# hank-kuo-cs/Volumetric-Primitives-Net

Measured on NVIDIA B200. Metric: primitive-loss fwd+bwd samples/sec, higher is better.
Workload: dtype f32

## Files before the change

### volumetric-primitives-net_b200/csrc/chamfer_tiled.cu

```cuda
#include <cstdlib>
#include <mutex>
#include <type_traits>
#include "common.cuh"

namespace vpn {

enum { MODE_EXACT = 0, MODE_DIFF = 1, MODE_EXPAND = 2, MODE_TC = 3 };

constexpr int kTThreads = 256;
constexpr int kTWarps = kTThreads / 32;
constexpr int kCW = 128;
constexpr int kMaxChunksPerSplit = 64;
constexpr float kBig = 1.0e30f;

__device__ __forceinline__ u64 pk(float a, float b) { u64 r; asm("mov.b64 %0, {%1,%2};" : "=l"(r) : "f"(a), "f"(b)); return r; }
__device__ __forceinline__ void upk(u64 v, float& a, float& b) { asm("mov.b64 {%0,%1}, %2;" : "=f"(a), "=f"(b) : "l"(v)); }
__device__ __forceinline__ u64 add2(u64 a, u64 b) { u64 r; asm("add.rn.f32x2 %0, %1, %2;" : "=l"(r) : "l"(a), "l"(b)); return r; }
__device__ __forceinline__ u64 sub2(u64 a, u64 b) { u64 r; asm("sub.rn.f32x2 %0, %1, %2;" : "=l"(r) : "l"(a), "l"(b)); return r; }
__device__ __forceinline__ u64 mul2(u64 a, u64 b) { u64 r; asm("mul.rn.f32x2 %0, %1, %2;" : "=l"(r) : "l"(a), "l"(b)); return r; }
__device__ __forceinline__ u64 fma2(u64 a, u64 b, u64 c) { u64 r; asm("fma.rn.f32x2 %0, %1, %2, %3;" : "=l"(r) : "l"(a), "l"(b), "l"(c)); return r; }
__device__ __forceinline__ float min3f(float a, float b, float c) { float r; asm("min.f32 %0, %1, %2, %3;" : "=f"(r) : "f"(a), "f"(b), "f"(c)); return r; }
__device__ __forceinline__ float warp_min_f32(float a) { float r; asm volatile("redux.sync.min.f32 %0, %1, 0xffffffff;" : "=f"(r) : "f"(a)); return r; }
__device__ __forceinline__ float inf_f() { return __int_as_float(0x7f800000); }

__device__ __forceinline__ float thr_of(float x, float rel, float abs_) {
  return __fadd_ru(__fmaf_ru(fabsf(x), rel, x), abs_);
}
__device__ __forceinline__ float mode_rel(int mode) {
  return mode == MODE_EXACT ? 9.5367431640625e-07f
       : mode == MODE_DIFF ? 3.814697265625e-06f
                           : 3.0517578125e-05f;
}

__device__ __forceinline__ float exact_d2s(float ax, float ay, float az, float bx, float by, float bz) {
  float dx = __fsub_rn(ax, bx), dy = __fsub_rn(ay, by), dz = __fsub_rn(az, bz);
  return __fadd_rn(__fadd_rn(__fmul_rn(dx, dx), __fmul_rn(dy, dy)), __fmul_rn(dz, dz));
}

template <int R>
struct TiledSmem {
  float4 tile[2][kCW];
  float colw[2][kTWarps][kCW];
  float rs_best[R][kTThreads];
  float rs_thr[R][kTThreads];
  u64 rs_mask[R][kTThreads];
  float red[kTWarps][4];
  float ctr[4];
};

template <int MODE>
__device__ __forceinline__ u64 pair_val(u64 c0, u64 c1, u64 c2, u64 c3, const float4& col, float one) {
  if (MODE == MODE_EXPAND) {
    u64 e = fma2(c0, pk(col.x, col.x), c3);
    e = fma2(c1, pk(col.y, col.y), e);
    e = fma2(c2, pk(col.z, col.z), e);
    return add2(e, pk(col.w, col.w));
  }
  u64 dx = sub2(c0, pk(col.x, col.x)), dy = sub2(c1, pk(col.y, col.y)), dz = sub2(c2, pk(col.z, col.z));
  if (MODE == MODE_EXACT) {
    u64 xx = mul2(dx, dx), yy = mul2(dy, dy), zz = mul2(dz, dz);
    u64 o2 = pk(one, one);
    return fma2(fma2(xx, o2, yy), o2, zz);
  }
  return fma2(dz, dz, fma2(dy, dy, mul2(dx, dx)));
}

template <int R, int MODE>
__global__ void __launch_bounds__(kTThreads, (R <= 8 ? 2 : 1))
chamfer_tiled_kernel(const float* __restrict__ p1, const float* __restrict__ p2,
                     float* __restrict__ rbest, u64* __restrict__ rmask,
                     float* __restrict__ cbest, unsigned* __restrict__ cmask,
                     float2* __restrict__ tslack, int* __restrict__ fallback,
                     int P, int M, int nchunks, int cps, float one, int only_flagged) {
  constexpr int TM = kTThreads * R;
  extern __shared__ __align__(16) unsigned char smem_raw[];
  TiledSmem<R>& sm = *reinterpret_cast<TiledSmem<R>*>(smem_raw);
  const int tid = threadIdx.x, lane = tid & 31, warp = tid >> 5;
  const int tile_i = blockIdx.x, split = blockIdx.y, b = blockIdx.z;
  const int ntiles = gridDim.x, nsplit = gridDim.y;
  if (only_flagged && fallback[b] == 0) return;
  const float* A = p1 + (size_t)b * P * 3;
  const float* T = p2 + (size_t)b * M * 3;

  u64 c0[R / 2], c1[R / 2], c2[R / 2], c3[R / 2];
  float rm[R];
  float cx = 0.f, cy = 0.f, cz = 0.f;
  float slack_rel = mode_rel(MODE), slack_abs = 1e-36f;
  {
    float x[R], y[R], z[R];
#pragma unroll
    for (int r = 0; r < R; ++r) {
      int i = min(tile_i * TM + r * kTThreads + tid, P - 1);
      x[r] = A[3 * (size_t)i]; y[r] = A[3 * (size_t)i + 1]; z[r] = A[3 * (size_t)i + 2];
    }
    if (MODE == MODE_EXPAND) {
      float sx = 0.f, sy = 0.f, sz = 0.f;
#pragma unroll
      for (int r = 0; r < R; ++r) { sx += x[r]; sy += y[r]; sz += z[r]; }
      sx = warp_sum(sx); sy = warp_sum(sy); sz = warp_sum(sz);
      if (lane == 0) { sm.red[warp][0] = sx; sm.red[warp][1] = sy; sm.red[warp][2] = sz; }
      __syncthreads();
      if (tid < 3) {
        float s = 0.f;
#pragma unroll
        for (int w = 0; w < kTWarps; ++w) s += sm.red[w][tid];
        sm.ctr[tid] = s / (float)TM;
      }
      __syncthreads();
      cx = sm.ctr[0]; cy = sm.ctr[1]; cz = sm.ctr[2];
      float rho2 = 0.f;
#pragma unroll
      for (int r = 0; r < R; ++r) {
        x[r] = __fsub_rn(x[r], cx); y[r] = __fsub_rn(y[r], cy); z[r] = __fsub_rn(z[r], cz);
        rho2 = fmaxf(rho2, fmaf(z[r], z[r], fmaf(y[r], y[r], x[r] * x[r])));
      }
#pragma unroll
      for (int o = 16; o > 0; o >>= 1) rho2 = fmaxf(rho2, __shfl_xor_sync(0xffffffffu, rho2, o));
      __syncthreads();
      if (lane == 0) sm.red[warp][3] = rho2;
      __syncthreads();
      rho2 = sm.red[0][3];
#pragma unroll
      for (int w = 1; w < kTWarps; ++w) rho2 = fmaxf(rho2, sm.red[w][3]);
      if (!(rho2 < kBig)) { if (tid == 0) atomicOr(&fallback[b], 1); rho2 = 0.f; }
      slack_abs = __fmaf_ru(8.0e-5f, rho2, 1e-36f);
    }
#pragma unroll
    for (int rp = 0; rp < R / 2; ++rp) {
      const int r0 = 2 * rp, r1 = 2 * rp + 1;
      if (MODE == MODE_EXPAND) {
        c0[rp] = pk(-2.f * x[r0], -2.f * x[r1]); c1[rp] = pk(-2.f * y[r0], -2.f * y[r1]); c2[rp] = pk(-2.f * z[r0], -2.f * z[r1]);
        c3[rp] = pk(fmaf(z[r0], z[r0], fmaf(y[r0], y[r0], x[r0] * x[r0])), fmaf(z[r1], z[r1], fmaf(y[r1], y[r1], x[r1] * x[r1])));
      } else {
        c0[rp] = pk(x[r0], x[r1]); c1[rp] = pk(y[r0], y[r1]); c2[rp] = pk(z[r0], z[r1]); c3[rp] = 0ull;
      }
    }
  }
  if (tid == 0 && split == 0) tslack[(size_t)b * ntiles + tile_i] = make_float2(slack_rel, slack_abs);
#pragma unroll
  for (int r = 0; r < R; ++r) {
    rm[r] = inf_f();
    sm.rs_best[r][tid] = inf_f(); sm.rs_thr[r][tid] = inf_f(); sm.rs_mask[r][tid] = 0ull;
  }
  const int c_first = split * cps;
  const int c_last = min(nchunks, c_first + cps);

  auto make_col = [&](float tx, float ty, float tz) -> float4 {
    if (MODE == MODE_EXPAND) {
      float x = __fsub_rn(tx, cx), y = __fsub_rn(ty, cy), z = __fsub_rn(tz, cz);
      float c = fmaf(z, z, fmaf(y, y, x * x));
      if (!(c < kBig)) atomicOr(&fallback[b], 1);
      return make_float4(x, y, z, c);
    }
    return make_float4(tx, ty, tz, 0.f);
  };

  if (tid < kCW) {
    int col = min(c_first * kCW + tid, M - 1);
    sm.tile[0][tid] = make_col(T[3 * (size_t)col], T[3 * (size_t)col + 1], T[3 * (size_t)col + 2]);
  }
  __syncthreads();

  for (int c = c_first; c < c_last; ++c) {
    const int buf = (c - c_first) & 1;
    float nx = 0.f, ny = 0.f, nz = 0.f;
    const bool has_next = (c + 1 < c_last) && (tid < kCW);
    if (has_next) {
      int col = min((c + 1) * kCW + tid, M - 1);
      nx = T[3 * (size_t)col]; ny = T[3 * (size_t)col + 1]; nz = T[3 * (size_t)col + 2];
    }
    const float4* tl = sm.tile[buf];
    float* cw = sm.colw[buf][warp];
#pragma unroll 2
    for (int k = 0; k < kCW; k += 2) {
      const float4 q0 = tl[k], q1 = tl[k + 1];
      float cm0 = inf_f(), cm1 = inf_f();
#pragma unroll
      for (int rp = 0; rp < R / 2; ++rp) {
        u64 d0 = pair_val<MODE>(c0[rp], c1[rp], c2[rp], c3[rp], q0, one);
        u64 d1 = pair_val<MODE>(c0[rp], c1[rp], c2[rp], c3[rp], q1, one);
        float a0, b0, a1, b1;
        upk(d0, a0, b0); upk(d1, a1, b1);
        rm[2 * rp] = min3f(rm[2 * rp], a0, a1);
        rm[2 * rp + 1] = min3f(rm[2 * rp + 1], b0, b1);
        cm0 = min3f(cm0, a0, b0);
        cm1 = min3f(cm1, a1, b1);
      }
      float w0 = warp_min_f32(cm0), w1 = warp_min_f32(cm1);
      if (lane == 0) *reinterpret_cast<float2*>(cw + k) = make_float2(w0, w1);
    }
    const u64 bit = 1ull << (c - c_first);
#pragma unroll
    for (int r = 0; r < R; ++r) {
      const float m = rm[r];
      rm[r] = inf_f();
      if (m <= sm.rs_thr[r][tid]) {
        const float best = sm.rs_best[r][tid];
        const float tm = thr_of(m, slack_rel, slack_abs);
        u64 mask = (tm < best) ? 0ull : sm.rs_mask[r][tid];
        sm.rs_mask[r][tid] = mask | bit;
        if (m < best) { sm.rs_best[r][tid] = m; sm.rs_thr[r][tid] = tm; }
      }
    }
    if (has_next) sm.tile[buf ^ 1][tid] = make_col(nx, ny, nz);
    __syncthreads();
    if (tid < kCW) {
      const int col = c * kCW + tid;
      if (col < M) {
        float w[kTWarps];
        float best = inf_f();
#pragma unroll
        for (int i = 0; i < kTWarps; ++i) { w[i] = sm.colw[buf][i][tid]; best = fminf(best, w[i]); }
        const float t = thr_of(best, slack_rel, slack_abs);
        unsigned mask = 0;
#pragma unroll
        for (int i = 0; i < kTWarps; ++i) mask |= (w[i] <= t) ? (1u << i) : 0u;
        size_t o = ((size_t)b * ntiles + tile_i) * M + col;
        cbest[o] = best; cmask[o] = mask;
      }
    }
  }
#pragma unroll
  for (int r = 0; r < R; ++r) {
    int row = tile_i * TM + r * kTThreads + tid;
    if (row < P) {
      size_t o = ((size_t)b * nsplit + split) * P + row;
      rbest[o] = sm.rs_best[r][tid]; rmask[o] = sm.rs_mask[r][tid];
    }
  }
}

constexpr int kRecThreads = 1024;
constexpr int kSegChunks = 64;
constexpr int kItemCap = 4096;

struct ExactBest {
  float d, hi, v; int i;
  __device__ __forceinline__ void init() { d = inf_f(); hi = inf_f(); v = inf_f(); i = 0x7fffffff; }
  __device__ __forceinline__ void offer(float dd, int idx) {
    if (dd <= hi) {
      float vv = sqrtf(dd);
      if (vv < v || (vv == v && idx < i)) { v = vv; i = idx; }
      if (dd < d) { d = dd; hi = thr_of(dd, 9.5367431640625e-07f, 1e-36f); }
    }
  }
  __device__ __forceinline__ u64 key() const { return ((u64)__float_as_uint(v) << 32) | (unsigned)i; }
};

__device__ __forceinline__ int unit_scan(const float (&d)[32], float dm, int rot, int* at) {
  if (!(dm < inf_f())) {
    bool any = false;
#pragma unroll
    for (int kk = 0; kk < 32; ++kk) any |= (d[kk] == inf_f());
    if (!any) return 0;
    return 2;
  }
  const float hi = thr_of(dm, 9.5367431640625e-07f, 1e-36f);
  int cnt = 0, pos = 0;
#pragma unroll
  for (int kk = 0; kk < 32; ++kk) {
    const bool in = d[kk] <= hi;
    cnt += in ? 1 : 0;
    pos += in ? kk : 0;
  }
  *at = (pos + rot) & 31;
  return cnt == 1 ? 1 : 2;
}

__device__ __noinline__ u64 unit_exact_walk(float ax, float ay, float az, const float4* __restrict__ pts, int idx0, int use_w) {
  ExactBest eb; eb.init();
  for (int k = 0; k < 32; ++k) {
    const float4 q = pts[k];
    eb.offer(exact_d2s(ax, ay, az, q.x, q.y, q.z), use_w ? __float_as_int(q.w) : idx0 + k);
  }
  return eb.i != 0x7fffffff ? eb.key() : ~0ull;
}

template <int NT>
__device__ __forceinline__ int block_exclusive_scan(int cnt, int* warp_sums, int* total) {
  const int lane = threadIdx.x & 31, warp = threadIdx.x >> 5;
  int inc = cnt;
#pragma unroll
  for (int o = 1; o < 32; o <<= 1) { int t = __shfl_up_sync(0xffffffffu, inc, o); if (lane >= o) inc += t; }
  if (lane == 31) warp_sums[warp] = inc;
  __syncthreads();
  if (warp == 0) {
    int w = lane < NT / 32 ? warp_sums[lane] : 0;
    int winc = w;
#pragma unroll
    for (int o = 1; o < 32; o <<= 1) { int t = __shfl_up_sync(0xffffffffu, winc, o); if (lane >= o) winc += t; }
    warp_sums[lane] = winc - w;
    if (lane == 31) warp_sums[32] = winc;
  }
  __syncthreads();
  int off = warp_sums[warp] + inc - cnt;
  *total = warp_sums[32];
  __syncthreads();
  return off;
}

__device__ __forceinline__ u64 expand_chunk_bits16(unsigned v) {
  u64 x = v & 0xffffu;
  x = (x | (x << 24)) & 0x000000ff000000ffull;
  x = (x | (x << 12)) & 0x000f000f000f000full;
  x = (x | (x << 6)) & 0x0303030303030303ull;
  x = (x | (x << 3)) & 0x1111111111111111ull;
  return x * 0xfull;
}
__device__ __forceinline__ void or_shifted256(u64 (&seg)[4], u64 w, int base) {
  if (w == 0ull || base >= 256 || base <= -64) return;
  const int k = base >> 6, sh = base & 63;
#pragma unroll
  for (int kk = 0; kk < 4; ++kk) {
    if (kk == k) seg[kk] |= w << sh;
    if (sh != 0 && kk == k + 1) seg[kk] |= w >> (64 - sh);
  }
}

constexpr int kRowGroup = kRecThreads / 2;
constexpr int kRowItemCap = kItemCap / 2;
constexpr size_t kRowsFixedSmem = (size_t)kRecThreads * (16 + 8 + 32 + 4 + 12 + 4) + (size_t)kItemCap * 4;
__device__ __forceinline__ void group_sync(int bar) { asm volatile("bar.sync %0, %1;" :: "r"(bar), "n"(kRowGroup) : "memory"); }
__device__ __forceinline__ int group_exclusive_scan(int cnt, int* warp_sums, int* total, int gt, int bar) {
  const int lane = gt & 31, warp = gt >> 5;
  int inc = cnt;
#pragma unroll
  for (int o = 1; o < 32; o <<= 1) { int t = __shfl_up_sync(0xffffffffu, inc, o); if (lane >= o) inc += t; }
  if (lane == 31) warp_sums[warp] = inc;
  group_sync(bar);
  if (warp == 0) {
    int w = lane < kRowGroup / 32 ? warp_sums[lane] : 0;
    int winc = w;
#pragma unroll
    for (int o = 1; o < 32; o <<= 1) { int t = __shfl_up_sync(0xffffffffu, winc, o); if (lane >= o) winc += t; }
    if (lane < kRowGroup / 32) warp_sums[lane] = winc - w;
    if (lane == 31) warp_sums[kRowGroup / 32] = winc;
  }
  group_sync(bar);
  int off = warp_sums[warp] + inc - cnt;
  *total = warp_sums[kRowGroup / 32];
  group_sync(bar);
  return off;
}

__global__ void __launch_bounds__(kRecThreads, 1)
chamfer_recover_rows_kernel(const float* __restrict__ p1, const float* __restrict__ p2, const float4* __restrict__ p2v, int mpad,
                            const float* __restrict__ rbest, const u64* __restrict__ rmask, int planes, size_t plane_stride,
                            const float2* __restrict__ tslack, float* __restrict__ min1, int* __restrict__ idx1,
                            int P, int M, int nchunks, int nsplit, int cps, int TM, int ntiles,
                            const int* __restrict__ skip, int nblk, int nitems, const int* __restrict__ rperm) {
  extern __shared__ __align__(16) unsigned char smem_raw[];
  float4* rowc_ = reinterpret_cast<float4*>(smem_raw);
  u64* key_ = reinterpret_cast<u64*>(rowc_ + kRecThreads);
  u64 (*pre_mask)[kRecThreads] = reinterpret_cast<u64 (*)[kRecThreads]>(key_ + kRecThreads);
  unsigned* items_ = reinterpret_cast<unsigned*>(pre_mask + 4);
  float* pre_rb = reinterpret_cast<float*>(items_ + kItemCap);
  float* pre_p1 = pre_rb + kRecThreads;
  int* pre_perm = reinterpret_cast<int*>(pre_p1 + 3 * kRecThreads);
  float4* cols = reinterpret_cast<float4*>(smem_raw + kRowsFixedSmem);
  __shared__ int warp_sums_[2][kRowGroup / 32 + 1];
  const int tid = threadIdx.x, lane = tid & 31, grp = tid / kRowGroup, gt = tid % kRowGroup, bar = 1 + grp;
  const bool use_pre = (nsplit == 1) && (planes == 4);
  auto prefetch = [&](int b_, int wi_) {
    const int row_ = (wi_ - b_ * nblk) * kRowGroup + gt;
    if (row_ < P) {
      const size_t o_ = (size_t)b_ * P + row_;
      cp_async4(&pre_rb[tid], rbest + o_);
#pragma unroll
      for (int w = 0; w < 4; ++w) cp_async8(&pre_mask[w][tid], rmask + o_ + w * plane_stride);
#pragma unroll
      for (int k = 0; k < 3; ++k) cp_async4(&pre_p1[tid * 3 + k], p1 + 3 * o_ + k);
      if (rperm) cp_async4(&pre_perm[tid], rperm + o_);
    }
    asm volatile("cp.async.commit_group;" ::: "memory");
  };
  float4* rowc = rowc_ + grp * kRowGroup; u64* key = key_ + grp * kRowGroup;
  unsigned* items = items_ + grp * kRowItemCap; int* warp_sums = warp_sums_[grp];
  const int per = (nitems + gridDim.x - 1) / gridDim.x;
  const int w0 = blockIdx.x * per, w1 = min(nitems, w0 + per);
  const int nseg = (nchunks + kSegChunks - 1) / kSegChunks;
  const float qnan = __int_as_float(0x7fc00000);
  for (int b = w0 / nblk; b * nblk < w1; ++b) {
    if (skip && skip[b]) continue;
    const int i0 = max(w0, b * nblk), i1 = min(w1, (b + 1) * nblk);
    for (int seg = 0; seg < nseg; ++seg) {
      const int seg_chunks = min(kSegChunks, nchunks - seg * kSegChunks);
      __syncthreads();
      if (p2v) {
        const float4* src = p2v + (size_t)b * mpad + (size_t)seg * kSegChunks * kCW;
        for (int i = tid; i < seg_chunks * kCW; i += kRecThreads) cols[i] = src[i];
      } else {
        const float* T = p2 + (size_t)b * M * 3;
        for (int i = tid; i < seg_chunks * kCW; i += kRecThreads) {
          const int col = seg * kSegChunks * kCW + i;
          cols[i] = col < M ? make_float4(T[3 * (size_t)col], T[3 * (size_t)col + 1], T[3 * (size_t)col + 2], __int_as_float(col))
                            : make_float4(qnan, qnan, qnan, __int_as_float(0x7fffffff));
        }
      }
      __syncthreads();
      if (use_pre && i0 + grp < i1) prefetch(b, i0 + grp);
      for (int wi = i0 + grp; wi < i1; wi += 2) {
        const int row = (wi - b * nblk) * kRowGroup + gt;
        const bool valid = row < P;
        auto orow_of = [&]() { return (size_t)b * P + (use_pre ? __float_as_int(rowc[gt].w) : (rperm ? rperm[(size_t)b * P + row] : row)); };
        float g = inf_f(), gthr = inf_f();
        u64 kinit = ~0ull;
        u64 sg[4] = {0ull, 0ull, 0ull, 0ull};
        if (use_pre) {
          asm volatile("cp.async.wait_all;" ::: "memory");
          if (valid) {
            rowc[gt] = make_float4(pre_p1[tid * 3], pre_p1[tid * 3 + 1], pre_p1[tid * 3 + 2], __int_as_float(rperm ? pre_perm[tid] : row));
            g = pre_rb[tid];
            if (seg > 0) { const size_t orow = orow_of(); kinit = ((u64)__float_as_uint(min1[orow]) << 32) | (unsigned)idx1[orow]; }
            const int rel = -seg * kSegChunks * 4;
            if (rel == 0) {
#pragma unroll
              for (int w = 0; w < 4; ++w) sg[w] = pre_mask[w][tid];
            } else {
#pragma unroll
              for (int w = 0; w < 4; ++w) or_shifted256(sg, pre_mask[w][tid], rel + 64 * w);
            }
          }
          if (wi + 2 < i1) prefetch(b, wi + 2);
          if (valid && seg_chunks < kSegChunks) {
            const int nu = seg_chunks * 4;
#pragma unroll
            for (int w = 0; w < 4; ++w) {
              const int left = nu - 64 * w;
              if (left <= 0) sg[w] = 0ull; else if (left < 64) sg[w] &= (1ull << left) - 1ull;
            }
          }
        } else if (valid) {
          const float* a = p1 + 3 * ((size_t)b * P + row);
          rowc[gt] = make_float4(a[0], a[1], a[2], 0.f);
          for (int s = 0; s < nsplit; ++s) g = fminf(g, rbest[((size_t)b * nsplit + s) * P + row]);
          const float2 sl = tslack[(size_t)b * ntiles + row / TM];
          gthr = thr_of(g, sl.x, sl.y);
          if (seg > 0) { const size_t orow = orow_of(); kinit = ((u64)__float_as_uint(min1[orow]) << 32) | (unsigned)idx1[orow]; }
          for (int s = 0; s < nsplit; ++s) {
            const size_t o = ((size_t)b * nsplit + s) * P + row;
            if (!(rbest[o] <= gthr)) continue;
            const int rel = (s * cps - seg * kSegChunks) * 4;
            if (planes == 4) {
#pragma unroll
              for (int w = 0; w < 4; ++w) or_shifted256(sg, rmask[o + w * plane_stride], rel + 64 * w);
            } else {
              const u64 m = rmask[o];
#pragma unroll
              for (int w = 0; w < 4; ++w) or_shifted256(sg, expand_chunk_bits16((unsigned)(m >> (16 * w))), rel + 64 * w);
            }
          }
          if (seg_chunks < kSegChunks) {
            const int nu = seg_chunks * 4;
#pragma unroll
            for (int w = 0; w < 4; ++w) {
              const int left = nu - 64 * w;
              if (left <= 0) sg[w] = 0ull; else if (left < 64) sg[w] &= (1ull << left) - 1ull;
            }
          }
        }
        key[gt] = kinit;
        int total;
        const int cnt = __popcll(sg[0]) + __popcll(sg[1]) + __popcll(sg[2]) + __popcll(sg[3]);
        const int off = group_exclusive_scan(cnt, warp_sums, &total, gt, bar);
        for (int base = 0; base < total; base += kRowItemCap) {
          int j = off;
#pragma unroll
          for (int w = 0; w < 4; ++w)
            for (u64 mm = sg[w]; mm; mm &= mm - 1, ++j)
              if (j >= base && j < base + kRowItemCap) items[j - base] = ((unsigned)gt << 8) | (unsigned)(64 * w + __ffsll((long long)mm) - 1);
          group_sync(bar);
          const int units = min(kRowItemCap, total - base);
          for (int it = gt; it < units; it += kRowGroup) {
            const unsigned item = items[it];
            const int r = item >> 8, u = item & 255;
            const float4 rc = rowc[r];
            const float4* src = cols + u * 32;
            float d[32], dm = inf_f();
#pragma unroll
            for (int kk = 0; kk < 32; ++kk) {
              const float4 q = src[(kk + lane) & 31];
              d[kk] = exact_d2s(rc.x, rc.y, rc.z, q.x, q.y, q.z);
              dm = fminf(dm, d[kk]);
            }
            int at;
            const int st = unit_scan(d, dm, lane, &at);
            if (st == 1) atomicMin(&key[r], ((u64)__float_as_uint(sqrtf(dm)) << 32) | (unsigned)__float_as_int(src[at].w));
            else if (st == 2) { const u64 kv = unit_exact_walk(rc.x, rc.y, rc.z, src, 0, 1); if (kv != ~0ull) atomicMin(&key[r], kv); }
          }
          group_sync(bar);
        }
        if (valid) {
          const u64 kv = key[gt];
          const size_t orow = orow_of();
          min1[orow] = __uint_as_float((unsigned)(kv >> 32));
          idx1[orow] = (int)(unsigned)(kv & 0xffffffffu);
        }
        group_sync(bar);
      }
    }
  }
}

__global__ void chamfer_col_thr_kernel(const float* __restrict__ cbest, const float2* __restrict__ tslack,
                                       float* __restrict__ cthr, int M, int ntiles) {
  const int b = blockIdx.y;
  const int col = blockIdx.x * blockDim.x + threadIdx.x;
  if (col >= M) return;
  float g = inf_f(), rel = 0.f, ab = 0.f;
  for (int ti = 0; ti < ntiles; ++ti) {
    g = fminf(g, cbest[((size_t)b * ntiles + ti) * M + col]);
    const float2 sl = tslack[(size_t)b * ntiles + ti];
    rel = fmaxf(rel, sl.x); ab = fmaxf(ab, sl.y);
  }
  cthr[(size_t)b * M + col] = thr_of(g, rel, ab);
}

template <int R, bool TC, int NT>
__global__ void __launch_bounds__(NT, 1024 / NT)
chamfer_recover_cols_kernel(const float* __restrict__ p1, const float* __restrict__ p2,
                            const float* __restrict__ cbest, const void* __restrict__ cmask_,
                            const float* __restrict__ cthr, u64* __restrict__ key2, int P, int M, int ntiles,
                            const int* __restrict__ skip, const int* __restrict__ rperm) {
  constexpr int TM = TC ? 128 * R : kTThreads * R;
  constexpr int kSub = TC ? 1 : ((R >= 4) ? 4 : R);
  constexpr int kRunsPerSub = TC ? 1 : R / kSub;
  constexpr int kPer = TC ? 4096 / NT : 8;
  constexpr int kBitBits = TC ? 6 : 4;
  using mask_t = typename std::conditional<TC, u64, unsigned>::type;
  const mask_t* __restrict__ cmask = reinterpret_cast<const mask_t*>(cmask_);
  const mask_t kBitMask = TC ? (mask_t)((4 * R >= 64) ? ~0ull : ((1ull << (4 * R)) - 1ull)) : (mask_t)0xffu;
  if (skip && skip[blockIdx.y]) return;
  extern __shared__ __align__(16) unsigned char smem_raw[];
  float4* rows = reinterpret_cast<float4*>(smem_raw);
  __shared__ unsigned items[kItemCap];
  __shared__ int warp_sums[33];
  const int b = blockIdx.y, ti = blockIdx.x, tid = threadIdx.x, lane = tid & 31;
  const float* A = p1 + (size_t)b * P * 3;
  const float qnan = __int_as_float(0x7fc00000);
  for (int i = tid; i < TM; i += NT) {
    int rowi = ti * TM + i;
    rows[i] = rowi < P ? make_float4(A[3 * (size_t)rowi], A[3 * (size_t)rowi + 1], A[3 * (size_t)rowi + 2],
                                     __int_as_float(rperm ? rperm[(size_t)b * P + rowi] : rowi))
                       : make_float4(qnan, qnan, qnan, __int_as_float(0x7fffffff));
  }
  const size_t rec0 = ((size_t)b * ntiles + ti) * M;
  for (int slab = 0; slab < M; slab += NT * kPer) {
    mask_t mk[kPer];
    int cnt = 0;
#pragma unroll
    for (int u = 0; u < kPer; ++u) {
      const int col = slab + u * NT + tid;
      mk[u] = 0;
      if (col < M && cbest[rec0 + col] <= cthr[(size_t)b * M + col]) mk[u] = cmask[rec0 + col] & kBitMask;
      cnt += TC ? __popcll((u64)mk[u]) : __popc((unsigned)mk[u]);
    }
    int total;
    const int off = block_exclusive_scan<NT>(cnt, warp_sums, &total);
    for (int base = 0; base < total; base += kItemCap) {
      int j = off;
#pragma unroll
      for (int u = 0; u < kPer; ++u)
        for (mask_t mm = mk[u]; mm; mm &= mm - 1, ++j)
          if (j >= base && j < base + kItemCap)
            items[j - base] = ((unsigned)(u * NT + tid) << kBitBits) |
                              (unsigned)((TC ? __ffsll((long long)mm) : __ffs((int)mm)) - 1);
      __syncthreads();
      const int units = min(kItemCap, total - base) * kSub;
      for (int it = tid; it < units; it += NT) {
        const unsigned item = items[it / kSub];
        const int col = slab + (int)(item >> kBitBits), w = item & ((1u << kBitBits) - 1u), sub = it % kSub;
        const float* t = p2 + 3 * ((size_t)b * M + col);
        const float tx = __ldg(t), ty = __ldg(t + 1), tz = __ldg(t + 2);
        u64 best = ~0ull;
#pragma unroll 1
        for (int rr = sub * kRunsPerSub; rr < (sub + 1) * kRunsPerSub; ++rr) {
          const int base_row = TC ? (w * 32) : (rr * kTThreads + w * 32);
          float d[32], dm = inf_f();
#pragma unroll
          for (int kk = 0; kk < 32; ++kk) {
            const float4 a = rows[base_row + ((kk + lane) & 31)];
            d[kk] = exact_d2s(a.x, a.y, a.z, tx, ty, tz);
            dm = fminf(dm, d[kk]);
          }
          int at;
          const int st = unit_scan(d, dm, lane, &at);
          u64 kv = ~0ull;
          if (st == 1) kv = ((u64)__float_as_uint(sqrtf(dm)) << 32) | (unsigned)__float_as_int(rows[base_row + at].w);
          else if (st == 2) kv = unit_exact_walk(tx, ty, tz, rows + base_row, 0, 1);
          best = kv < best ? kv : best;
        }
        if (best != ~0ull) atomicMin(&key2[(size_t)b * M + col], best);
      }
      __syncthreads();
    }
  }
}

__global__ void chamfer_unpack_key_kernel(const u64* __restrict__ key, float* __restrict__ mn, int* __restrict__ idx, size_t n,
                                          const int* __restrict__ skip, int per_sample, const int* __restrict__ perm) {
  size_t i = (size_t)blockIdx.x * blockDim.x + threadIdx.x;
  if (i >= n) return;
  const size_t smp = i / (size_t)per_sample;
  if (skip && skip[smp]) return;
  u64 k = key[i];
  const size_t o = perm ? smp * (size_t)per_sample + (size_t)perm[i] : i;
  mn[o] = __uint_as_float((unsigned)(k >> 32));
  idx[o] = (int)(unsigned)(k & 0xffffffffu);
}

struct TiledPlan { int R, ntiles, nchunks, nsplit, cps, tc, TM; };

size_t chamfer_tc_smem_bytes(int NB);
int chamfer_tc_plan_words();
int chamfer_tc_launch(const float* p1, const float* p2, float* rbest, u64* rmask, float* cbest, u64* cmask,
                      float2* tslack, int* fallback, float* tmax, const float* cbox, const float* rbox, const float* rthr,
                      const float* cub, u64* stats, unsigned* plan_masks, int* plan_work, int* plan_order, int with_bounds,
                      int B, int P, int M, int NB, int ntiles, int nsplit, int nchunks, int cps, cudaStream_t s);
int chamfer_prep_launch(const float* p1, const float* p2, float* p2s, float4* p2v, int* perm, float* cbox, float* rbox, float* rthr,
                        float* cub, float* tmax, float* p1s, int* rperm, unsigned long long* stats, int B, int P, int M, cudaStream_t s);
int chamfer_flagged_launch(const float* p1, const float* p2, float* min1, int* idx1, float* min2, int* idx2,
                           const int* fallback, int B, int P, int M, cudaStream_t s);

static void finish_plan(TiledPlan& pl, int B, long long slots, int min_cps) {
  long long base = (long long)pl.ntiles * B;
  long long s = (4 * slots + base - 1) / base;
  long long smin = (pl.nchunks + kMaxChunksPerSplit - 1) / kMaxChunksPerSplit;
  long long smax = pl.nchunks / min_cps;
  if (s > smax) s = smax;
  if (s < smin) s = smin;
  if (s > pl.nchunks) s = pl.nchunks;
  if (s < 1) s = 1;
  pl.cps = (int)((pl.nchunks + s - 1) / s);
  pl.nsplit = (pl.nchunks + pl.cps - 1) / pl.cps;
}

static bool make_plan(int B, int P, int M, int sm_count, TiledPlan& pl) {
  if (P < 1024 || M < kCW || B < 1) return false;
  pl.tc = 0;
  pl.nchunks = (M + kCW - 1) / kCW;
  const int rs[3] = {16, 8, 4};
  int pick = 4;
  for (int k = 0; k < 3; ++k) {
    int R = rs[k], tm = kTThreads * R;
    long long nt = (P + tm - 1) / tm;
    double waste = (double)(nt * tm) / P;
    long long slots = (long long)sm_count * (R <= 8 ? 2 : 1);
    if (waste <= 1.26 && nt * B * pl.nchunks >= 2 * slots) { pick = R; break; }
  }
  { int r = tuning_value(kTuneTiledR); if (r == 4 || r == 8 || r == 16) pick = r; }
  pl.R = pick;
  pl.TM = kTThreads * pl.R;
  pl.ntiles = (P + pl.TM - 1) / pl.TM;
  finish_plan(pl, B, (long long)sm_count * (pl.R <= 8 ? 2 : 1), 1);
  return pl.nsplit <= 65535;
}

static bool make_plan_tc(int B, int P, int M, int sm_count, TiledPlan& pl) {
  if (P < 512 || M < kCW || B < 1) return false;
  pl.tc = 1;
  pl.nchunks = (M + kCW - 1) / kCW;
  const int nbs[3] = {16, 8, 4};
  int pick = 4;
  for (int k = 0; k < 3; ++k) {
    int nb = nbs[k], tm = 128 * nb;
    long long nt = (P + tm - 1) / tm;
    double waste = (double)(nt * tm) / P;
    if (waste <= 1.26 && nt * B * pl.nchunks >= 2LL * sm_count * 8) { pick = nb; break; }
  }
  { int r = tuning_value(kTuneTcNb); if (r == 4 || r == 8 || r == 16) pick = r; }
  pl.R = pick;
  pl.TM = 128 * pl.R;
  pl.ntiles = (P + pl.TM - 1) / pl.TM;
  finish_plan(pl, B, sm_count, 4);
  return pl.nsplit <= 65535;
}

static size_t al256(size_t x) { return (x + 255) & ~(size_t)255; }

struct TiledWs { size_t rbest, rmask, cbest, cmask, tslack, fallback, tmax, cthr, key2, p2s, p2v, perm, cbox, rbox, rthr, cub, pmask, pwork, porder, p1s, rperm, total; };
static TiledWs ws_layout(int B, int P, int M, const TiledPlan& pl) {
  TiledWs w; size_t o = 0;
  w.rbest = o; o += al256((size_t)B * pl.nsplit * P * 4);
  w.rmask = o; o += al256((size_t)B * pl.nsplit * P * 8 * (pl.tc ? 4 : 1));
  w.cbest = o; o += al256((size_t)B * pl.ntiles * M * 4);
  w.cmask = o; o += al256((size_t)B * pl.ntiles * M * (pl.tc ? 8 : 4));
  w.tslack = o; o += al256((size_t)B * pl.ntiles * 8);
  w.fallback = o; o += al256((size_t)B * 4 + 8 + 128);
  w.tmax = o; o += al256((size_t)B * 4);
  w.cthr = o; o += al256((size_t)B * M * 4);
  w.key2 = o; o += al256((size_t)B * M * 8);
  w.p2s = w.p2v = w.perm = w.cbox = w.rbox = w.rthr = w.cub = w.pmask = w.pwork = w.porder = w.p1s = w.rperm = 0;
  if (pl.tc) {
    const size_t nrb = (size_t)(P + 127) / 128;
    w.p2s = o; o += al256((size_t)B * M * 12);
    w.p2v = o; o += al256((size_t)B * pl.nchunks * kCW * 16);
    w.perm = o; o += al256((size_t)B * M * 4);
    w.cbox = o; o += al256((size_t)B * pl.nchunks * 32);
    w.rbox = o; o += al256((size_t)B * nrb * 32);
    w.rthr = o; o += al256((size_t)B * nrb * 4);
    w.cub = o; o += al256((size_t)B * pl.nchunks * 4);
    const size_t ncta = (size_t)pl.ntiles * pl.nsplit * B;
    w.pmask = o; o += al256(ncta * (size_t)chamfer_tc_plan_words() * 4);
    w.pwork = o; o += al256(ncta * 4);
    w.porder = o; o += al256(ncta * 4);
    w.p1s = o; o += al256((size_t)B * P * 12);
    w.rperm = o; o += al256((size_t)B * P * 4);
  }
  w.total = o;
  return w;
}

static bool plan_for(int mode, int B, int P, int M, TiledPlan& pl) {
  const int kPlanSms = device_sm_count();
  if (mode == MODE_TC) return make_plan_tc(B, P, M, kPlanSms, pl);
  if (mode >= 0) return make_plan(B, P, M, kPlanSms, pl);
  return make_plan_tc(B, P, M, kPlanSms, pl) || make_plan(B, P, M, kPlanSms, pl);
}

int chamfer_tiled_supported(int B, int P, int M, int mode) {
  TiledPlan pl;
  return plan_for(mode, B, P, M, pl) ? 1 : 0;
}

int chamfer_tiled_uses_tc(int B, int P, int M, int mode) {
  TiledPlan pl;
  return (plan_for(mode, B, P, M, pl) && pl.tc) ? 1 : 0;
}

size_t chamfer_tiled_workspace_bytes(int B, int P, int M, int mode) {
  TiledPlan pl;
  if (!plan_for(mode, B, P, M, pl)) return 0;
  return ws_layout(B, P, M, pl).total;
}

int chamfer_tiled_stats(int B, int P, int M, int mode, const void* ws_, unsigned long long* out, cudaStream_t s) {
  TiledPlan pl;
  for (int i = 0; i < 16; ++i) out[i] = 0;
  if (!plan_for(mode, B, P, M, pl) || !pl.tc) return VPN_OK;
  TiledWs wl = ws_layout(B, P, M, pl);
  const char* src = reinterpret_cast<const char*>(ws_) + wl.fallback + (((size_t)B * 4 + 7) & ~(size_t)7);
  if (cudaMemcpyAsync(out, src, 128, cudaMemcpyDeviceToHost, s) != cudaSuccess || cudaStreamSynchronize(s) != cudaSuccess) {
    vpn_set_error("chamfer stats: copy failed"); return VPN_ERR_CUDA;
  }
  return VPN_OK;
}

template <int R, int MODE>
static int launch_main(const float* p1, const float* p2, char* ws, const TiledWs& wl, const TiledPlan& pl,
                       int B, int P, int M, int only_flagged, cudaStream_t s) {
  static DeviceOnce once;
  size_t smem = sizeof(TiledSmem<R>);
  {
    cudaError_t e = set_dyn_smem(chamfer_tiled_kernel<R, MODE>, (int)smem, once);
    if (e != cudaSuccess) { vpn_set_error("chamfer tiled: smem attribute: %s", cudaGetErrorString(e)); return VPN_ERR_CUDA; }
  }
  dim3 grid(pl.ntiles, pl.nsplit, B);
  chamfer_tiled_kernel<R, MODE><<<grid, kTThreads, smem, s>>>(
      p1, p2, reinterpret_cast<float*>(ws + wl.rbest), reinterpret_cast<u64*>(ws + wl.rmask),
      reinterpret_cast<float*>(ws + wl.cbest), reinterpret_cast<unsigned*>(ws + wl.cmask),
      reinterpret_cast<float2*>(ws + wl.tslack), reinterpret_cast<int*>(ws + wl.fallback),
      P, M, pl.nchunks, pl.cps, 1.0f, only_flagged);
  return vpn_check_launch("chamfer_tiled_kernel");
}

template <int R>
static int launch_main_mode(int mode, const float* p1, const float* p2, char* ws, const TiledWs& wl, const TiledPlan& pl,
                            int B, int P, int M, int only_flagged, cudaStream_t s) {
  switch (mode) {
    case MODE_EXACT: return launch_main<R, MODE_EXACT>(p1, p2, ws, wl, pl, B, P, M, only_flagged, s);
    case MODE_DIFF:  return launch_main<R, MODE_DIFF>(p1, p2, ws, wl, pl, B, P, M, only_flagged, s);
    default:         return launch_main<R, MODE_EXPAND>(p1, p2, ws, wl, pl, B, P, M, only_flagged, s);
  }
}

static int launch_any(int mode, const float* p1, const float* p2, char* ws, const TiledWs& wl, const TiledPlan& pl,
                      int B, int P, int M, int only_flagged, cudaStream_t s) {
  switch (pl.R) {
    case 16: return launch_main_mode<16>(mode, p1, p2, ws, wl, pl, B, P, M, only_flagged, s);
    case 8:  return launch_main_mode<8>(mode, p1, p2, ws, wl, pl, B, P, M, only_flagged, s);
    default: return launch_main_mode<4>(mode, p1, p2, ws, wl, pl, B, P, M, only_flagged, s);
  }
}

template <int R, bool TC>
static int launch_recover_cols(const float* p1, const float* p2, const float* cb, const void* cmk, const float* cthr,
                               u64* key2, int B, int P, int M, int ntiles, const int* skip, const int* rperm, cudaStream_t s) {
  static DeviceOnce once, once_half;
  const size_t smem = (size_t)(TC ? 128 * R : kTThreads * R) * sizeof(float4);
  if (TC && (long long)ntiles * B >= 2LL * device_sm_count()) {
    if (set_dyn_smem(chamfer_recover_cols_kernel<R, TC, 512>, (int)smem, once_half) != cudaSuccess) {
      vpn_set_error("chamfer tiled: smem attribute (cols recovery)"); return VPN_ERR_CUDA;
    }
    chamfer_recover_cols_kernel<R, TC, 512><<<dim3(ntiles, B), 512, smem, s>>>(p1, p2, cb, cmk, cthr, key2, P, M, ntiles, skip, rperm);
    return vpn_check_launch("chamfer_recover_cols_kernel");
  }
  if (set_dyn_smem(chamfer_recover_cols_kernel<R, TC, kRecThreads>, (int)smem, once) != cudaSuccess) {
    vpn_set_error("chamfer tiled: smem attribute (cols recovery)"); return VPN_ERR_CUDA;
  }
  chamfer_recover_cols_kernel<R, TC, kRecThreads><<<dim3(ntiles, B), kRecThreads, smem, s>>>(p1, p2, cb, cmk, cthr, key2, P, M, ntiles, skip, rperm);
  return vpn_check_launch("chamfer_recover_cols_kernel");
}

struct SideStream { cudaStream_t s = nullptr; cudaEvent_t fork = nullptr, join = nullptr; bool ok = false; std::mutex mu; };
static SideStream g_side[64];
static SideStream* side_stream_for(cudaStream_t s) {
  int dev = 0;
  if (cudaGetDevice(&dev) != cudaSuccess || dev < 0 || dev >= 64) return nullptr;
  SideStream& ss = g_side[dev];
  if (ss.ok) return &ss;
  cudaStreamCaptureStatus st = cudaStreamCaptureStatusNone;
  if (cudaStreamIsCapturing(s, &st) != cudaSuccess || st != cudaStreamCaptureStatusNone) { cudaGetLastError(); return nullptr; }
  std::lock_guard<std::mutex> lock(ss.mu);
  if (!ss.ok) {
    if (cudaStreamCreateWithFlags(&ss.s, cudaStreamNonBlocking) != cudaSuccess ||
        cudaEventCreateWithFlags(&ss.fork, cudaEventDisableTiming) != cudaSuccess ||
        cudaEventCreateWithFlags(&ss.join, cudaEventDisableTiming) != cudaSuccess) { cudaGetLastError(); return nullptr; }
    ss.ok = true;
  }
  return &ss;
}

int chamfer_tiled_fwd(const float* p1, const float* p2, float* min1, int* idx1, float* min2, int* idx2,
                      int B, int P, int M, void* ws_, size_t ws_bytes, int mode, cudaStream_t s, cudaEvent_t* ev) {
  TiledPlan pl;
  if (!plan_for(mode, B, P, M, pl)) { vpn_set_error("chamfer tiled: unsupported shape"); return VPN_ERR_SHAPE; }
  if (mode < 0) mode = pl.tc ? MODE_TC : MODE_EXPAND;
  TiledWs wl = ws_layout(B, P, M, pl);
  if (ws_bytes < wl.total) { vpn_set_error("chamfer tiled: workspace too small (%zu < %zu)", ws_bytes, wl.total); return VPN_ERR_WORKSPACE; }
  char* ws = reinterpret_cast<char*>(ws_);
  int* fallback = reinterpret_cast<int*>(ws + wl.fallback);
  const int* skip = nullptr;
  int rc;
  if (ev) cudaEventRecord(ev[0], s);
  const size_t flag_bytes = (((size_t)B * 4 + 7) & ~(size_t)7) + 128;
  if (mode == MODE_EXPAND || mode == MODE_TC) {
    if (cudaMemsetAsync(fallback, 0, flag_bytes, s) != cudaSuccess) { vpn_set_error("chamfer tiled: memset failed"); return VPN_ERR_CUDA; }
  }
  const float* p2w = p2;
  const int* perm = nullptr;
  const float4* p2v = nullptr;
  const float* p1w = p1;
  const int* rperm = nullptr;
  if (mode == MODE_TC) {
    float* p2s = reinterpret_cast<float*>(ws + wl.p2s);
    int* pm = reinterpret_cast<int*>(ws + wl.perm);
    float* cbox = reinterpret_cast<float*>(ws + wl.cbox); float* rbox = reinterpret_cast<float*>(ws + wl.rbox);
    float* rthr = reinterpret_cast<float*>(ws + wl.rthr); float* cub = reinterpret_cast<float*>(ws + wl.cub);
    float* tmax = reinterpret_cast<float*>(ws + wl.tmax);
    u64* stats = reinterpret_cast<u64*>(ws + wl.fallback + (((size_t)B * 4 + 7) & ~(size_t)7));
    const bool prune = tuning_value(kTuneTcPrune) != 2;
    if (prune) {
      float4* pv = reinterpret_cast<float4*>(ws + wl.p2v);
      float* p1s = reinterpret_cast<float*>(ws + wl.p1s);
      int* rp = reinterpret_cast<int*>(ws + wl.rperm);
      if ((rc = chamfer_prep_launch(p1, p2, p2s, pv, pm, cbox, rbox, rthr, cub, tmax, p1s, rp, stats, B, P, M, s))) return rc;
      p2w = p2s; perm = pm; p2v = pv; p1w = p1s; rperm = rp;
    }
    rc = chamfer_tc_launch(p1w, p2w, reinterpret_cast<float*>(ws + wl.rbest), reinterpret_cast<u64*>(ws + wl.rmask),
                           reinterpret_cast<float*>(ws + wl.cbest), reinterpret_cast<u64*>(ws + wl.cmask),
                           reinterpret_cast<float2*>(ws + wl.tslack), fallback, tmax, prune ? cbox : nullptr, rbox, rthr, cub, stats,
                           reinterpret_cast<unsigned*>(ws + wl.pmask), reinterpret_cast<int*>(ws + wl.pwork),
                           reinterpret_cast<int*>(ws + wl.porder), prune ? 0 : 1, B, P, M, pl.R, pl.ntiles, pl.nsplit, pl.nchunks,
                           pl.cps, s);
    if (rc) return rc;
    if (ev) cudaEventRecord(ev[1], s);
    if ((rc = chamfer_flagged_launch(p1, p2, min1, idx1, min2, idx2, fallback, B, P, M, s))) return rc;
    skip = fallback;
  } else {
    if ((rc = launch_any(mode, p1, p2, ws, wl, pl, B, P, M, 0, s))) return rc;
    if (ev) cudaEventRecord(ev[1], s);
    if (mode == MODE_EXPAND) {
      if ((rc = launch_any(MODE_DIFF, p1, p2, ws, wl, pl, B, P, M, 1, s))) return rc;
    }
  }
  if (ev) cudaEventRecord(ev[2], s);
  SideStream* side = tuning_value(kTuneSerialRecovery) ? nullptr : side_stream_for(s);
  std::unique_lock<std::mutex> side_lock;
  cudaStream_t sc = s;
  if (side) {
    side_lock = std::unique_lock<std::mutex>(side->mu);
    if (cudaEventRecord(side->fork, s) == cudaSuccess && cudaStreamWaitEvent(side->s, side->fork, 0) == cudaSuccess) sc = side->s;
    else { cudaGetLastError(); side = nullptr; side_lock.unlock(); }
  }
  {
    static DeviceOnce once_rows;
    const size_t smem_rows = kRowsFixedSmem + (size_t)(pl.nchunks < kSegChunks ? pl.nchunks : kSegChunks) * kCW * sizeof(float4);
    if (set_dyn_smem(chamfer_recover_rows_kernel, (int)(kRowsFixedSmem + kSegChunks * kCW * sizeof(float4)), once_rows) != cudaSuccess) {
      vpn_set_error("chamfer tiled: smem attribute (rows recovery)"); return VPN_ERR_CUDA;
    }
    const int nblk = (P + kRowGroup - 1) / kRowGroup;
    const long long nitems = (long long)nblk * B;
    if (nitems > 0x7fffffffLL) { vpn_set_error("chamfer tiled: too many row blocks"); return VPN_ERR_SHAPE; }
    const int sms = device_sm_count();
    chamfer_recover_rows_kernel<<<(unsigned)(nitems < sms ? nitems : sms), kRecThreads, smem_rows, s>>>(
        p1w, p2w, p2v, pl.nchunks * kCW, reinterpret_cast<const float*>(ws + wl.rbest), reinterpret_cast<const u64*>(ws + wl.rmask),
        pl.tc ? 4 : 1, (size_t)B * pl.nsplit * P, reinterpret_cast<const float2*>(ws + wl.tslack), min1, idx1, P, M, pl.nchunks,
        pl.nsplit, pl.cps, pl.TM, pl.ntiles, skip, nblk, (int)nitems, rperm);
    if ((rc = vpn_check_launch("chamfer_recover_rows_kernel"))) return rc;
  }
  if (ev) cudaEventRecord(ev[3], s);
  const float* cb = reinterpret_cast<const float*>(ws + wl.cbest);
  const void* cmk = ws + wl.cmask;
  const float2* tsl = reinterpret_cast<const float2*>(ws + wl.tslack);
  float* cthr = reinterpret_cast<float*>(ws + wl.cthr);
  u64* key2 = reinterpret_cast<u64*>(ws + wl.key2);
  if (cudaMemsetAsync(key2, 0xFF, (size_t)B * M * 8, sc) != cudaSuccess) { vpn_set_error("chamfer tiled: memset failed"); return VPN_ERR_CUDA; }
  chamfer_col_thr_kernel<<<dim3((M + 255) / 256, B), 256, 0, sc>>>(cb, tsl, cthr, M, pl.ntiles);
  if ((rc = vpn_check_launch("chamfer_col_thr_kernel"))) return rc;
  if (pl.tc) {
    switch (pl.R) {
      case 16: rc = launch_recover_cols<16, true>(p1w, p2w, cb, cmk, cthr, key2, B, P, M, pl.ntiles, skip, rperm, sc); break;
      case 8:  rc = launch_recover_cols<8, true>(p1w, p2w, cb, cmk, cthr, key2, B, P, M, pl.ntiles, skip, rperm, sc); break;
      default: rc = launch_recover_cols<4, true>(p1w, p2w, cb, cmk, cthr, key2, B, P, M, pl.ntiles, skip, rperm, sc); break;
    }
  } else {
    switch (pl.R) {
      case 16: rc = launch_recover_cols<16, false>(p1, p2, cb, cmk, cthr, key2, B, P, M, pl.ntiles, skip, nullptr, sc); break;
      case 8:  rc = launch_recover_cols<8, false>(p1, p2, cb, cmk, cthr, key2, B, P, M, pl.ntiles, skip, nullptr, sc); break;
      default: rc = launch_recover_cols<4, false>(p1, p2, cb, cmk, cthr, key2, B, P, M, pl.ntiles, skip, nullptr, sc); break;
    }
  }
  if (rc) return rc;
  {
    size_t n = (size_t)B * M;
    chamfer_unpack_key_kernel<<<(unsigned)((n + 255) / 256), 256, 0, sc>>>(key2, min2, idx2, n, skip, M, perm);
  }
  rc = vpn_check_launch("chamfer_unpack_key_kernel");
  if (side) {
    if (cudaEventRecord(side->join, sc) != cudaSuccess || cudaStreamWaitEvent(s, side->join, 0) != cudaSuccess) {
      vpn_set_error("chamfer tiled: stream join failed"); rc = VPN_ERR_CUDA;
    }
  }
  if (ev) cudaEventRecord(ev[4], s);
  return rc;
}

}
```

Measured before the change: 34460.

## Add owner-per-block row recovery kernel that stages candidate units in shared memory

Adds a new row-recovery kernel in which each 128-thread block owns 128 sorted rows. It gathers the union of candidate 32-point units flagged by the masks, stages those units in shared memory in batches, and distributes row-unit work items across the threads. Per-row nearest keys are reduced with shared atomicMin. The aim is to cut redundant global loads of target points and balance uneven per-row candidate counts. It only runs when there are enough blocks to fill the GPU, and in exchange it adds scans, multiple passes over the masks and shared-memory atomic contention.

```diff
diff --git a/volumetric-primitives-net_b200/csrc/chamfer_tiled.cu b/volumetric-primitives-net_b200/csrc/chamfer_tiled.cu
--- a/volumetric-primitives-net_b200/csrc/chamfer_tiled.cu
+++ b/volumetric-primitives-net_b200/csrc/chamfer_tiled.cu
@@ -609,6 +609,156 @@
   idx[o] = (int)(unsigned)(k & 0xffffffffu);
 }
 
+constexpr int kOwn = 128;
+constexpr int kStageUnits = 32;
+constexpr int kOwnItemCap = 1024;
+constexpr int kOwnCtasPerSm = 8;
+
+struct OwnedSmem {
+  float4 pts[kStageUnits * 32];
+  float4 own[kOwn];
+  u64 key[kOwn];
+  unsigned items[kOwnItemCap];
+  int sunit[kStageUnits];
+  int warp_sums[33];
+};
+constexpr size_t kMaxOwnedSmem = 96 * 1024;
+static size_t owned_smem_bytes(int nunits) { const size_t nw = ((size_t)nunits + 31) / 32; return sizeof(OwnedSmem) + nw * 4 + (nw + 1) * 4; }
+
+template <class ForEach, class Load>
+__device__ __forceinline__ void owned_recover(OwnedSmem& sm, unsigned* uni, int* wpre, int nw, const ForEach& for_each, const Load& load) {
+  const int tid = threadIdx.x, lane = tid & 31;
+  for (int i = tid; i < nw; i += kOwn) uni[i] = 0u;
+  sm.key[tid] = ~0ull;
+  __syncthreads();
+  int cnt_all = 0;
+  for_each([&](int u) { atomicOr(&uni[u >> 5], 1u << (u & 31)); ++cnt_all; });
+  __syncthreads();
+  if (tid < 32) {
+    int carry = 0;
+    for (int w0 = 0; w0 < nw; w0 += 32) {
+      const int w = w0 + lane;
+      const int c = w < nw ? __popc(uni[w]) : 0;
+      int inc = c;
+#pragma unroll
+      for (int o = 1; o < 32; o <<= 1) { const int t = __shfl_up_sync(0xffffffffu, inc, o); if (lane >= o) inc += t; }
+      if (w < nw) wpre[w] = carry + inc - c;
+      carry += __shfl_sync(0xffffffffu, inc, 31);
+    }
+    if (lane == 0) wpre[nw] = carry;
+  }
+  __syncthreads();
+  const int nu = wpre[nw];
+  auto slot_of = [&](int u) { return wpre[u >> 5] + __popc(uni[u >> 5] & ((1u << (u & 31)) - 1u)); };
+  for (int p0 = 0; p0 < nu; p0 += kStageUnits) {
+    const int p1 = min(nu, p0 + kStageUnits);
+    if (tid < 32) {
+      for (int w = lane; w < nw; w += 32) {
+        if (wpre[w] >= p1 || wpre[w + 1] <= p0) continue;
+        int s = wpre[w];
+        for (unsigned m = uni[w]; m; m &= m - 1u, ++s)
+          if (s >= p0 && s < p1) sm.sunit[s - p0] = 32 * w + __ffs((int)m) - 1;
+      }
+    }
+    __syncthreads();
+    for (int i = tid; i < (p1 - p0) * 32; i += kOwn) sm.pts[i] = load(sm.sunit[i >> 5], i & 31);
+    int cnt = cnt_all;
+    if (nu > kStageUnits) {
+      cnt = 0;
+      for_each([&](int u) { const int s = slot_of(u); cnt += (s >= p0 && s < p1) ? 1 : 0; });
+    }
+    int total;
+    const int off = block_exclusive_scan<kOwn>(cnt, sm.warp_sums, &total);
+    for (int base = 0; base < total; base += kOwnItemCap) {
+      int j = off;
+      for_each([&](int u) {
+        const int s = slot_of(u);
+        if (s >= p0 && s < p1) {
+          if (j >= base && j < base + kOwnItemCap) sm.items[j - base] = ((unsigned)tid << 8) | (unsigned)(s - p0);
+          ++j;
+        }
+      });
+      __syncthreads();
+      const int n = min(kOwnItemCap, total - base);
+      for (int it = tid; it < n; it += kOwn) {
+        const unsigned item = sm.items[it];
+        const int r = item >> 8;
+        const float4 rc = sm.own[r];
+        const float4* src = sm.pts + (item & 255u) * 32;
+        float d[32], dm = inf_f();
+#pragma unroll
+        for (int kk = 0; kk < 32; ++kk) {
+          const float4 q = src[(kk + lane) & 31];
+          d[kk] = exact_d2s(rc.x, rc.y, rc.z, q.x, q.y, q.z);
+          dm = fminf(dm, d[kk]);
+        }
+        int at;
+        const int st = unit_scan(d, dm, lane, &at);
+        if (st == 1) atomicMin(&sm.key[r], ((u64)__float_as_uint(sqrtf(dm)) << 32) | (unsigned)__float_as_int(src[at].w));
+        else if (st == 2) { const u64 kv = unit_exact_walk(rc.x, rc.y, rc.z, src, 0, 1); if (kv != ~0ull) atomicMin(&sm.key[r], kv); }
+      }
+      __syncthreads();
+    }
+  }
+}
+
+__global__ void __launch_bounds__(kOwn, kOwnCtasPerSm)
+chamfer_recover_rows_sorted_kernel(const float* __restrict__ p1s, const float4* __restrict__ p2v, int mpad,
+                                   const float* __restrict__ rbest, const u64* __restrict__ rmask, size_t plane_stride,
+                                   const float2* __restrict__ tslack, float* __restrict__ min1, int* __restrict__ idx1,
+                                   int P, int nunits, int nsplit, int cps, int TM, int ntiles,
+                                   const int* __restrict__ skip, const int* __restrict__ rperm) {
+  extern __shared__ __align__(16) unsigned char smem_raw[];
+  OwnedSmem& sm = *reinterpret_cast<OwnedSmem*>(smem_raw);
+  const int nw = (nunits + 31) >> 5;
+  unsigned* uni = reinterpret_cast<unsigned*>(smem_raw + sizeof(OwnedSmem));
+  int* wpre = reinterpret_cast<int*>(uni + nw);
+  const int b = blockIdx.y, tid = threadIdx.x, row = blockIdx.x * kOwn + tid;
+  if (skip && skip[b]) return;
+  const bool valid = row < P;
+  const size_t orow = (size_t)b * P + row;
+  float gthr = inf_f();
+  u64 m1[4] = {0ull, 0ull, 0ull, 0ull};
+  if (valid) {
+    sm.own[tid] = make_float4(p1s[3 * orow], p1s[3 * orow + 1], p1s[3 * orow + 2], 0.f);
+    if (nsplit == 1) {
+#pragma unroll
+      for (int w = 0; w < 4; ++w) m1[w] = rmask[orow + w * plane_stride];
+    } else {
+      float g = inf_f();
+      for (int s = 0; s < nsplit; ++s) g = fminf(g, rbest[((size_t)b * nsplit + s) * P + row]);
+      const float2 sl = tslack[(size_t)b * ntiles + row / TM];
+      gthr = thr_of(g, sl.x, sl.y);
+    }
+  }
+  auto for_each = [&](auto&& f) {
+    if (!valid) return;
+    if (nsplit == 1) {
+#pragma unroll
+      for (int w = 0; w < 4; ++w)
+        for (u64 m = m1[w]; m; m &= m - 1) { const int u = 64 * w + __ffsll((long long)m) - 1; if (u < nunits) f(u); }
+      return;
+    }
+    for (int s = 0; s < nsplit; ++s) {
+      const size_t o = ((size_t)b * nsplit + s) * P + row;
+      if (!(rbest[o] <= gthr)) continue;
+      for (int w = 0; w < 4; ++w) {
+        const int u0 = s * cps * 4 + 64 * w;
+        for (u64 m = rmask[o + w * plane_stride]; m; m &= m - 1) { const int u = u0 + __ffsll((long long)m) - 1; if (u < nunits) f(u); }
+      }
+    }
+  };
+  const float4* tv = p2v + (size_t)b * mpad;
+  owned_recover(sm, uni, wpre, nw, for_each, [&](int u, int k) { return __ldg(tv + (size_t)u * 32 + k); });
+  if (valid) {
+    const u64 kv = sm.key[tid];
+    const size_t o = (size_t)b * P + rperm[orow];
+    min1[o] = __uint_as_float((unsigned)(kv >> 32));
+    idx1[o] = (int)(unsigned)(kv & 0xffffffffu);
+  }
+}
+
+
 struct TiledPlan { int R, ntiles, nchunks, nsplit, cps, tc, TM; };
 
 size_t chamfer_tc_smem_bytes(int NB);
@@ -883,7 +1033,21 @@
     if (cudaEventRecord(side->fork, s) == cudaSuccess && cudaStreamWaitEvent(side->s, side->fork, 0) == cudaSuccess) sc = side->s;
     else { cudaGetLastError(); side = nullptr; side_lock.unlock(); }
   }
-  {
+  const long long sorted_blocks = (long long)B * ((P + kOwn - 1) / kOwn);
+  if (p2v && sorted_blocks >= (long long)kOwnCtasPerSm * device_sm_count()) {
+    static DeviceOnce once_rows_sorted;
+    const int nunits = pl.nchunks * 4;
+    const size_t smem = owned_smem_bytes(nunits);
+    if (smem > kMaxOwnedSmem) { vpn_set_error("chamfer tiled: target cloud too large for the row recovery"); return VPN_ERR_SHAPE; }
+    if (set_dyn_smem(chamfer_recover_rows_sorted_kernel, (int)kMaxOwnedSmem, once_rows_sorted) != cudaSuccess) {
+      vpn_set_error("chamfer tiled: smem attribute (rows recovery)"); return VPN_ERR_CUDA;
+    }
+    chamfer_recover_rows_sorted_kernel<<<dim3((P + kOwn - 1) / kOwn, B), kOwn, smem, s>>>(
+        p1w, p2v, pl.nchunks * kCW, reinterpret_cast<const float*>(ws + wl.rbest), reinterpret_cast<const u64*>(ws + wl.rmask),
+        (size_t)B * pl.nsplit * P, reinterpret_cast<const float2*>(ws + wl.tslack), min1, idx1, P, nunits, pl.nsplit, pl.cps,
+        pl.TM, pl.ntiles, skip, rperm);
+    if ((rc = vpn_check_launch("chamfer_recover_rows_sorted_kernel"))) return rc;
+  } else {
     static DeviceOnce once_rows;
     const size_t smem_rows = kRowsFixedSmem + (size_t)(pl.nchunks < kSegChunks ? pl.nchunks : kSegChunks) * kCW * sizeof(float4);
     if (set_dyn_smem(chamfer_recover_rows_kernel, (int)(kRowsFixedSmem + kSegChunks * kCW * sizeof(float4)), once_rows) != cudaSuccess) {
```

New measurement: 35530, median of 6. 1.03x the previous value.
